# google-research/nerf-from-image

Measured on AMD Instinct MI355X. Metric: rendered rays/sec (128x128, 64+64 samples), higher is better.
Workload: dtype f32 (decoder MLP operands split-fp16 hi+lo, 22 bits; strict fp32: config.value_mlp_exact_fp32)

## Files before the change

### nerf_from_image_amd/csrc/nfi_kernels.hip

```cpp
#include "nfi_device.hpp"
#include "../../include/nfi_hip.h"
#include "nfi_host.hpp"

#include <algorithm>
#include <cstddef>
#include <cstdio>
#include <cstring>

using namespace nfi;

thread_local char nfi_err_buf[256] = "";
extern "C" const char* nfi_last_error(void) { return nfi_err_buf; }
extern "C" int nfi_version(void) { return 102; }


constexpr int kP2tPixels = 256, kP2tPitch = 288;
template <int TEX>
__global__ __launch_bounds__(256) void planes_to_texels_kernel(const float* __restrict__ planes, void* __restrict__ texels,
                                                               int hw) {
  __shared__ __attribute__((aligned(16))) float tile[kC][kP2tPitch];
  const int img = blockIdx.y;
  const int px0 = blockIdx.x * kP2tPixels;
  const float* src = planes + (size_t)img * kC * hw;
  {
// ... 1005 lines not shown
  const int64_t ray = (int64_t)blockIdx.x * 4 + wave;
  if (ray >= a.n_rays) return;
  WaveSlab& slab = slabs[wave];
  const int M = a.n_bins, K = a.n_samples;
  float bins[2], wts[2];
#pragma unroll
  for (int j = 0; j < 2; ++j) {
    int e = j * 64 + lane;
    bins[j] = e < M ? a.bins[ray * M + e] : 0.0f;
    wts[j] = e < M - 1 ? a.weights[ray * (M - 1) + e] : 0.0f;
  }
  build_cdf<2>(slab, bins, wts, M, lane);
#pragma unroll
  for (int j = 0; j < 2; ++j) {
    int e = j * 64 + lane;
    if (e < K) {
      float u = a.u[ray * a.u_row_stride + e];
      int ind;
      float z = invert_cdf<16>(slab, M, u, ind);
      a.samples[ray * K + e] = z;
      if (a.inds) a.inds[ray * K + e] = ind;
    }
    if (a.cdf && e < M) a.cdf[ray * M + e] = slab.cdf[e];
  }
}

extern "C" int nfi_sample_pdf(const nfi_sample_pdf_args* a, nfi_stream_t stream) {
  REQUIRE(a && a->bins && a->weights && a->u && a->samples, "sample_pdf: null pointer");
  REQUIRE(a->n_rays > 0 && a->n_bins >= 2 && a->n_bins <= 128 && a->n_samples >= 1 && a->n_samples <= 128,
          "sample_pdf: need 2 <= bins <= 128 and 1 <= samples <= 128");
  hipLaunchKernelGGL(sample_pdf_kernel, dim3((unsigned)((a->n_rays + 3) / 4)), dim3(256), 0, (hipStream_t)stream, *a);
  return check_launch("sample_pdf");
}

__global__ __launch_bounds__(256) void resample_kernel(nfi_resample_args a) {
  __shared__ WaveSlab slabs[4];
  const int lane = lane_id();
  const int wave = threadIdx.x >> 6;
  const int64_t ray = (int64_t)blockIdx.x * 4 + wave;
  if (ray >= a.n_rays) return;
  WaveSlab& slab = slabs[wave];
  const int S = a.n_samples;
  float sigma = lane < S ? a.sigma[ray * S + lane] : 0.0f;
  float t = lane < S ? a.depth[ray * S + lane] : 0.0f;
  float u = lane < S ? a.u[ray * a.u_row_stride + lane] : 0.0f;
  float dn = norm3(a.ray_directions[ray * 3], a.ray_directions[ray * 3 + 1], a.ray_directions[ray * 3 + 2]);
  ResampleTaps taps;
  float z = resample_ray(slab, sigma, t, S, dn, u, lane, &taps);
  if (lane < S) {
    a.fine_depth[ray * S + lane] = z;
    if (a.weights) a.weights[ray * S + lane] = taps.w;
    if (a.smooth) a.smooth[ray * S + lane] = taps.smooth;
    if (a.inds) a.inds[ray * S + lane] = taps.ind;
  }
  if (a.cdf && lane < S - 1) a.cdf[ray * (S - 1) + lane] = slab.cdf[lane];
}

__global__ __launch_bounds__(256) void resample_wide_kernel(nfi_resample_args a) {
  __shared__ WaveSlab slabs[4];
  const int lane = lane_id();
  const int wave = threadIdx.x >> 6;
  const int64_t ray = (int64_t)blockIdx.x * 4 + wave;
  if (ray >= a.n_rays) return;
  WaveSlab& slab = slabs[wave];
  const int S = a.n_samples;
  float sigma[2], t[2], u[2], z[2], w[2], sm[2];
  int ind[2];
#pragma unroll
  for (int j = 0; j < 2; ++j) {
    const int e = j * 64 + lane;
    sigma[j] = e < S ? a.sigma[ray * S + e] : 0.0f;
    t[j] = e < S ? a.depth[ray * S + e] : 0.0f;
    u[j] = e < S ? a.u[ray * a.u_row_stride + e] : 0.0f;
  }
  float dn = norm3(a.ray_directions[ray * 3], a.ray_directions[ray * 3 + 1], a.ray_directions[ray * 3 + 2]);
  float Tc[2];
  resample_ray_wide<2>(slab, sigma, t, S, dn, u, lane, z, w, sm, ind, Tc);
#pragma unroll
  for (int j = 0; j < 2; ++j) {
    const int e = j * 64 + lane;
    if (e < S) {
      a.fine_depth[ray * S + e] = z[j];
      if (a.weights) a.weights[ray * S + e] = w[j];
      if (a.smooth) a.smooth[ray * S + e] = sm[j];
      if (a.inds) a.inds[ray * S + e] = ind[j];
    }
    if (a.cdf && e < S - 1) a.cdf[ray * (S - 1) + e] = slab.cdf[e];
  }
}

extern "C" int nfi_resample(const nfi_resample_args* a, nfi_stream_t stream) {
  REQUIRE(a && a->sigma && a->ray_directions && a->depth && a->u && a->fine_depth, "resample: null pointer");
  REQUIRE(a->n_rays > 0 && a->n_samples >= 4 && a->n_samples <= NFI_MAX_SAMPLES, "resample: n_samples must be in [4,128]");
  const dim3 grid((unsigned)((a->n_rays + 3) / 4));
  if (a->n_samples <= 64) hipLaunchKernelGGL(resample_kernel, grid, dim3(256), 0, (hipStream_t)stream, *a);
  else hipLaunchKernelGGL(resample_wide_kernel, grid, dim3(256), 0, (hipStream_t)stream, *a);
  return check_launch("resample");
}

template <int NS>
__global__ __launch_bounds__(256) void composite_kernel(nfi_composite_args a) {
  __shared__ WaveSlabT<64 * NS> slabs[4];
  const int lane = lane_id();
  const int wave = threadIdx.x >> 6;
  const int64_t ray = (int64_t)blockIdx.x * 4 + wave;
  if (ray >= a.n_rays) return;
  auto& slab = slabs[wave];
  const int na = a.n_a, nb = a.n_b, n = na + nb;
  float dep[NS], sig[NS], cr[NS], cg[NS], cb[NS];
  int eidx[NS];
#pragma unroll
  for (int j = 0; j < NS; ++j) {
    int e = j * 64 + lane;
    dep[j] = sig[j] = cr[j] = cg[j] = cb[j] = 0.0f;
    eidx[j] = e;
    if (e < na) {
      size_t i = (size_t)ray * na + e;
      dep[j] = a.depth_a[i]; sig[j] = a.sigma_a[i];
      cr[j] = a.rgb_a[i * 3]; cg[j] = a.rgb_a[i * 3 + 1]; cb[j] = a.rgb_a[i * 3 + 2];
    } else if (e < n) {
      size_t i = (size_t)ray * nb + (e - na);
      dep[j] = a.depth_b[i]; sig[j] = a.sigma_b[i];
      cr[j] = a.rgb_b[i * 3]; cg[j] = a.rgb_b[i * 3 + 1]; cb[j] = a.rgb_b[i * 3 + 2];
    }
  }
  int rank[NS];
  if (nb > 0) {
    merge_scatter<NS>(slab, dep, sig, cr, cg, cb, eidx, n, rank);
  } else {
#pragma unroll
    for (int j = 0; j < NS; ++j) {
      int e = j * 64 + lane;
      rank[j] = e;
      if (e < n) { slab.srt[0][e] = dep[j]; slab.srt[1][e] = sig[j]; slab.srt[2][e] = cr[j]; slab.srt[3][e] = cg[j]; slab.srt[4][e] = cb[j]; }
    }
    wave_lds_fence();
  }
  float dn = norm3(a.ray_directions[ray * 3], a.ray_directions[ray * 3 + 1], a.ray_directions[ray * 3 + 2]);
  float w[NS];
  CompositeOut o = composite_slab<NS>(slab, n, dn, a.white_background, lane, w);
  if (lane == 0) {
    a.rgb_map[ray * 3] = o.r; a.rgb_map[ray * 3 + 1] = o.g; a.rgb_map[ray * 3 + 2] = o.b;
    a.depth_map[ray] = o.depth;
    a.mask[ray] = o.mask;
  }
#pragma unroll
  for (int j = 0; j < NS; ++j) {
    int e = j * 64 + lane;
    if (e < n) {
      if (a.weights) a.weights[(size_t)ray * n + e] = w[j];
      if (a.depth_sorted) a.depth_sorted[(size_t)ray * n + e] = slab.srt[0][e];
      if (a.perm) a.perm[(size_t)ray * n + rank[j]] = e;
    }
  }
  if (a.n_extra > 0 && a.extra_map) {
    wave_lds_fence();
#pragma unroll
    for (int j = 0; j < NS; ++j) {
      int e = j * 64 + lane;
      if (e < n) slab.cdf[e] = w[j];
    }
    wave_lds_fence();
    float we[NS];
#pragma unroll
    for (int j = 0; j < NS; ++j) { int e = j * 64 + lane; we[j] = e < n ? slab.cdf[rank[j]] : 0.0f; }
    for (int c = 0; c < a.n_extra; ++c) {
      float acc = 0.0f;
#pragma unroll
      for (int j = 0; j < NS; ++j) {
        int e = j * 64 + lane;
        if (e < na) acc += we[j] * a.extra_a[((size_t)ray * na + e) * a.n_extra + c];
        else if (e < n) acc += we[j] * a.extra_b[((size_t)ray * nb + (e - na)) * a.n_extra + c];
      }
      acc = wave_sum(acc);
      if (lane == 0) a.extra_map[ray * a.n_extra + c] = acc;
    }
  }
}

extern "C" int nfi_composite_fwd(const nfi_composite_args* a, nfi_stream_t stream) {
  REQUIRE(a && a->ray_directions && a->depth_a && a->sigma_a && a->rgb_a && a->rgb_map && a->depth_map && a->mask,
          "composite: null pointer");
  REQUIRE(a->n_rays > 0 && a->n_a > 0 && a->n_b >= 0 && a->n_a + a->n_b <= NFI_MAX_SAMPLES_SINGLE_PASS,
          "composite: need 1 <= n_a + n_b <= 512");
  REQUIRE(a->n_b == 0 || (a->n_a <= NFI_MAX_SAMPLES && a->n_b <= NFI_MAX_SAMPLES), "composite: merged lists hold at most 128 samples each");
  REQUIRE(a->n_b == 0 || (a->depth_b && a->sigma_b && a->rgb_b), "composite: list b missing");
  REQUIRE(a->n_extra == 0 || (a->extra_a && (a->n_b == 0 || a->extra_b)), "composite: extra attribute missing");
  const dim3 grid((unsigned)((a->n_rays + 3) / 4));
  if (a->n_a + a->n_b <= 128) hipLaunchKernelGGL(composite_kernel<2>, grid, dim3(256), 0, (hipStream_t)stream, *a);
  else if (a->n_a + a->n_b <= 256) hipLaunchKernelGGL(composite_kernel<4>, grid, dim3(256), 0, (hipStream_t)stream, *a);
  else hipLaunchKernelGGL(composite_kernel<8>, grid, dim3(256), 0, (hipStream_t)stream, *a);
  return check_launch("composite_fwd");
}

#include "nfi_backward_rays.inc"
#include "nfi_regulariser.inc"
#include "nfi_neighbours.inc"
#include "nfi_handoff.inc"
#include "nfi_pnp.inc"
#include "nfi_viewdir_mapper.inc"

struct RenderKernelParams {
  int n_scenes, hw, S;
  int fine, white;
  float scene_range;
  const float* ro; const float* rd; const float* near_raw; const float* far_raw; const uint8_t* hit;
  const uint32_t* reduce;
  uint32_t* counter;
  int width;
  int tile_order;
  int xcd_blocks;
  uint32_t* xcd_counter;
  int xcd_block_shift;
  int fetch_batch;
  const void* texels; int res; int layout;
  const float* image; int A; const float* att;
  int use_sdf; const float* beta; const float* alpha;
  const float* noise_c; const float* noise_f; int64_t noise_f_stride;
  float* rgb; float* depth; float* mask;
  float* near_plane; float* far_plane;
  float* t_coarse; float* sigma_coarse; float* rgb_coarse;
  float* t_fine; float* sigma_fine; float* rgb_fine;
  float* t_sorted; float* weights; int32_t* perm;
  int skip_missed;
  unsigned long long* prof;
  const float* xray;
  float term_eps;
  float* semantics;
  float* coords;
  float* normals;
  unsigned long long* clock_probe;
  FastDiv div_scene_rays, div_bps, div_bw;
  int tap_stride;
  int stash;
};

struct ClockProbe {
  unsigned long long c0 = 0, r0 = 0;
  bool on = false;
  __device__ __forceinline__ void start(const RenderKernelParams& k) {
    on = k.clock_probe && blockIdx.x == 0 && threadIdx.x == 0;
    if (on) { c0 = __builtin_readcyclecounter(); r0 = __builtin_amdgcn_s_memrealtime(); }
  }
  __device__ __forceinline__ void stop(const RenderKernelParams& k) const {
    if (on) {
      k.clock_probe[0] = __builtin_readcyclecounter() - c0;
      k.clock_probe[1] = __builtin_amdgcn_s_memrealtime() - r0;
    }
  }
};

__device__ __forceinline__ float uniform_f32(float v) {
  return bits2f((uint32_t)__builtin_amdgcn_readfirstlane((int)f2bits(v)));
}

struct RayInputs {
  float ox, oy, oz, dx, dy, dz, near, far, noise, u;
  uint32_t hit;
};

struct RayQueue {
  const RenderKernelParams& k;
  int lane;
  uint32_t n_rays, xcd, bsh, bw, bps, n_blocks, q_cur, pos_next, pos_end, batch, tiles_x;
  bool dry;
  __device__ __forceinline__ RayQueue(const RenderKernelParams& kk, int l) : k(kk), lane(l) {
    n_rays = (uint32_t)k.n_scenes * (uint32_t)k.hw;
    xcd = k.xcd_blocks ? (__builtin_amdgcn_s_getreg(6164) & 7u) : 0u;
    bsh = (uint32_t)k.xcd_block_shift;
    bw = (uint32_t)k.width >> bsh;
    bps = bw * (((uint32_t)k.hw / (uint32_t)k.width) >> bsh);
    n_blocks = bps * (uint32_t)k.n_scenes;
    q_cur = xcd; pos_next = 0; pos_end = 0; dry = false;
    batch = (uint32_t)k.fetch_batch;
    tiles_x = (uint32_t)k.width >> 3;
  }
  __device__ __forceinline__ uint32_t ray_at(uint32_t q, uint32_t pos) const {
    const uint32_t b = (pos >> (2 * bsh)) * 8u + q;
    const uint32_t in = pos & ((1u << (2 * bsh)) - 1u), scene = fastdiv(b, k.div_bps), bb = b - scene * bps;
    const uint32_t by = fastdiv(bb, k.div_bw), bx = bb - by * bw;
    const uint32_t st = in >> 6, sty = st >> (bsh - 3), stx = st & ((1u << (bsh - 3)) - 1u);
    const uint32_t y = (by << bsh) + (sty << 3) + ((in >> 3) & 7u), x = (bx << bsh) + (stx << 3) + (in & 7u);
    return scene * (uint32_t)k.hw + y * (uint32_t)k.width + x;
  }
  __device__ __forceinline__ uint32_t fetch() {
    if (!k.xcd_blocks) {
      uint32_t p = 0;
      if (lane == 0) p = atomicAdd(k.counter, 1u);
      return (uint32_t)__builtin_amdgcn_readfirstlane((int)p);
    }
    if (pos_next == pos_end && !dry) {
      dry = true;
      for (uint32_t i = 0; i < 8; ++i) {
        uint32_t base = 0;
        if (lane == 0) base = atomicAdd(k.xcd_counter + q_cur * 16, batch);
        base = (uint32_t)__builtin_amdgcn_readfirstlane((int)base);
        if ((base >> (2 * bsh)) * 8u + q_cur < n_blocks) { pos_next = base; pos_end = base + batch; dry = false; break; }
        q_cur = (q_cur + 1) & 7u;
      }
    }
    if (dry) return n_rays;
    return ray_at(q_cur, pos_next++);
  }
  __device__ __forceinline__ uint32_t ray_of(uint32_t pos) const {
    if (k.xcd_blocks || !k.tile_order) return pos;
    const uint32_t scene = pos / (uint32_t)k.hw, p = pos - scene * (uint32_t)k.hw;
    const uint32_t tile = p >> 6, in = p & 63u;
    const uint32_t ty = tile / tiles_x, tx = tile - ty * tiles_x;
    return scene * (uint32_t)k.hw + ((ty << 3) + (in >> 3)) * (uint32_t)k.width + (tx << 3) + (in & 7u);
  }
};

constexpr int kRenderPlain = 0, kRenderTaps = 1, kRenderProf = 2, kRenderTerm = 3, kRenderExtra = 4, kRenderNormals = 5;
constexpr int kSemPitch = 2 * 64 + 4;
constexpr int kSemPitchWide = 2 * 128 + 8;
extern __shared__ __attribute__((aligned(16))) float nfi_dyn_lds[];

typedef __attribute__((address_space(3))) float lds_float;

template <int NS, class Slab>
__device__ __forceinline__ void composite_coords(const Slab& slab, const float (&w)[NS], int n, int lane, float ox, float oy,
                                                 float oz, float dx, float dy, float dz, float* out3) {
  float cx = 0.0f, cy = 0.0f, cz = 0.0f;
#pragma unroll
  for (int j = 0; j < NS; ++j) {
    const int e = j * 64 + lane;
    if (e < n) {
      const float t = slab.srt[0][e];
      cx += w[j] * (ox + dx * t); cy += w[j] * (oy + dy * t); cz += w[j] * (oz + dz * t);
    }
  }
  cx = wave_sum(cx); cy = wave_sum(cy); cz = wave_sum(cz);
  if (lane == 0) { out3[0] = cx; out3[1] = cy; out3[2] = cz; }
}


template <int PREC, int kImg>
__device__ __forceinline__ void stage_decoder_image(float* lds, const float* image) {
  if (PREC == 1) {
    for (int i = threadIdx.x; i < kB1F; i += blockDim.x) lds[i] = image[kW1H + i];
    for (int i = kB1F + threadIdx.x; i < kLdsImageFloats; i += blockDim.x) lds[i] = image[i];
  } else {
    for (int i = threadIdx.x; i < kImg; i += blockDim.x) lds[i] = image[i];
  }
  __syncthreads();
}

template <int TEX>
__device__ __forceinline__ void enter_scene(FieldParams& P, const RenderKernelParams& k, float* vf, int scene, int lane) {
  const size_t tb = TEX == 0 ? 128 : 64;
  const char* tex_scene = reinterpret_cast<const char*>(k.texels) + (size_t)scene * 3 * k.res * k.res * tb;
  P.rsrc = __builtin_amdgcn_make_buffer_rsrc(const_cast<char*>(tex_scene), 0, (int)P.scene_bytes, 0x00020000);
  wave_lds_fence();
  {
    int c = lane & 3, row = lane >> 2;
    float v = 0.0f;
    if (k.att && c < 3 && row >= 1 && row <= k.A) v = k.att[((size_t)scene * k.A + (row - 1)) * 3 + c];
    vf[lane] = v;
  }
  wave_lds_fence();
}

__device__ __forceinline__ void store_pixel(const RenderKernelParams& k, uint32_t ray, float r, float g, float b, float depth,
                                            float mask) {
  k.rgb[(size_t)ray * 3] = r; k.rgb[(size_t)ray * 3 + 1] = g; k.rgb[(size_t)ray * 3 + 2] = b;
  k.depth[ray] = depth; k.mask[ray] = mask;
}

__device__ __forceinline__ void store_sample_tap(float* t_out, float* sigma_out, float* rgb_out, size_t i, float t, float sigma,
                                                 float r, float g, float b) {
  if (t_out) t_out[i] = t;
  if (sigma_out) sigma_out[i] = sigma;
  if (rgb_out) { float* q = rgb_out + i * 3; q[0] = r; q[1] = g; q[2] = b; }
}

template <int NS, class Slab>
__device__ __forceinline__ void store_sorted_taps(const RenderKernelParams& k, const Slab& slab, const float (&w)[NS], uint32_t ray,
                                                  int n, int lane) {
#pragma unroll
  for (int j = 0; j < NS; ++j) {
    const int e = j * 64 + lane;
    if (e < n) {
      if (k.weights) k.weights[(size_t)ray * n + e] = w[j];
      if (k.t_sorted) k.t_sorted[(size_t)ray * n + e] = slab.srt[0][e];
    }
  }
}

template <bool NRM>
__device__ __forceinline__ void zero_missed_maps(const RenderKernelParams& k, uint32_t ray, int lane, float bg) {
  if (k.coords && lane < 3) k.coords[(size_t)ray * 3 + lane] = 0.0f;
  if (k.semantics && lane < k.A) k.semantics[(size_t)ray * k.A + lane] = 0.0f;
  if (NRM && lane < 3) k.normals[(size_t)ray * 3 + lane] = bg;
}

__device__ __forceinline__ void zero_stash_row(const RenderKernelParams& k, uint32_t ray, int S, int lane) {
  for (int e = lane; e < S; e += 64) {
    const size_t zs = (size_t)ray * (size_t)k.tap_stride + e;
    k.t_coarse[zs] = 0.0f; k.sigma_coarse[zs] = 0.0f;
    float* q = k.rgb_coarse + zs * 3; q[0] = 0.0f; q[1] = 0.0f; q[2] = 0.0f;
    if (k.fine) {
      k.t_fine[zs] = 0.0f; k.sigma_fine[zs] = 0.0f;
      q = k.rgb_fine + zs * 3; q[0] = 0.0f; q[1] = 0.0f; q[2] = 0.0f;
    }
  }
}

template <int TEX, bool ATT, int OCC, int MODE, int PREC, bool VD = false>
__global__ __launch_bounds__(256, OCC) void render_fwd_kernel(RenderKernelParams k) {
  constexpr bool TAPS = MODE == kRenderTaps, PROF = MODE == kRenderProf, TERM = MODE == kRenderTerm;
  constexpr bool EXTRA = MODE == kRenderExtra || MODE == kRenderNormals, NRM = MODE == kRenderNormals;
  constexpr int SEMP = (EXTRA && ATT) ? kSemPitch : 0;
  constexpr int kImg = VD ? kVdImageFloats : kLdsImageFloats;
  __shared__ __attribute__((aligned(16))) float lds[kImg];
  __shared__ __attribute__((aligned(16))) float vfs[4][64];
  __shared__ WaveSlab slabs[4];
  if constexpr (NRM) stage_normal_operands(nfi_dyn_lds, k.image, VD ? kVdW1F : kW1F, VD ? kVdW2 : kW2F);
  ClockProbe clock;
  clock.start(k);
  stage_decoder_image<PREC, kImg>(lds, k.image);
  const int lane = lane_id();
  const int wave = threadIdx.x >> 6;
  WaveSlab& slab = slabs[wave];
  float* vf = vfs[wave];
  const int S = k.S;
  const bool valid = lane < S;
  const float fill_near = ordered_key_inv(~k.reduce[0]), fill_far = ordered_key_inv(k.reduce[1]);
  const float bg = k.white ? 1.0f : 0.0f;
  const uint32_t n_rays = (uint32_t)k.n_scenes * (uint32_t)k.hw;

  FieldParams P = make_field_params(k.texels, k.res, TEX, k.A, k.use_sdf, k.beta, k.alpha, lds, kImg, k.layout);
  P.vf = vf;
  P.w1t = nfi_dyn_lds; P.w2r0 = nfi_dyn_lds + kW1TFloats;
  int cur_scene = -1;

  float* semT = nullptr;
  if constexpr (SEMP > 0) {
    if (k.semantics) {
      semT = nfi_dyn_lds + (NRM ? kNrmLdsFloats : 0) + wave * (k.A * kSemPitch);
      for (int i = lane; i < k.A * kSemPitch; i += 64) ((lds_float*)semT)[i] = 0.0f;
      wave_lds_fence();
    }
  }

  auto load_inputs = [&](uint32_t ray, RayInputs& in) {
    const size_t r3 = (size_t)ray * 3;
    in.hit = k.hit[ray];
    in.ox = k.ro[r3]; in.oy = k.ro[r3 + 1]; in.oz = k.ro[r3 + 2];
    in.dx = k.rd[r3]; in.dy = k.rd[r3 + 1]; in.dz = k.rd[r3 + 2];
    in.near = k.near_raw[ray]; in.far = k.far_raw[ray];
    in.noise = (k.noise_c && valid) ? k.noise_c[(size_t)ray * S + lane] : 0.0f;
    in.u = (k.fine && valid) ? k.noise_f[(size_t)ray * k.noise_f_stride + lane] : 0.0f;
  };

  RayQueue queue(k, lane);
  auto fetch = [&]() -> uint32_t { return queue.fetch(); };
  uint32_t cur = fetch(), nxt = fetch(), fly = 0;
  RayInputs in, pre;
  unsigned long long pc[12] = {0, 0, 0, 0, 0, 0, 0, 0, 0, 0, 0, 0};
  unsigned long long tk0 = PROF ? __builtin_readcyclecounter() : 0;
  if (cur < n_rays) load_inputs(queue.ray_of(cur), in);
  while (cur < n_rays) {
    if (nxt < n_rays) load_inputs(queue.ray_of(nxt), pre);
    const uint32_t ray = queue.ray_of(cur);
    const uint32_t hitb = in.hit;
    float out_r = bg, out_g = bg, out_b = bg, out_d = 0.0f, out_m = 0.0f;
    if (k.skip_missed && !(hitb & 2)) {
      if constexpr (EXTRA) zero_missed_maps<NRM>(k, ray, lane, bg);
      if constexpr (TAPS) {
        if (k.stash) zero_stash_row(k, ray, S, lane);
      }
    } else {
      unsigned long long t0 = PROF ? __builtin_readcyclecounter() : 0;
      const int scene = (int)fastdiv(ray, k.div_scene_rays);
      if (scene != cur_scene) {
        cur_scene = scene;
        enter_scene<TEX>(P, k, vf, scene, lane);
      }
      const float ox = in.ox, oy = in.oy, oz = in.oz, dx = in.dx, dy = in.dy, dz = in.dz;
      float near = in.near, far = in.far;
      finish_planes((hitb & 1) != 0, fill_near, fill_far, near, far);
      const float dnorm = norm3(dx, dy, dz);
      const size_t rs = (size_t)ray * (size_t)k.tap_stride;

      float tc = 0.0f;
      if (valid) tc = stratified_depth(near, far, lane, S, in.noise, k.noise_c != nullptr);
      MergeIn c;
      float ncx = 0.0f, ncy = 0.0f, ncz = 0.0f, nfx = 0.0f, nfy = 0.0f, nfz = 0.0f;
      unsigned long long t1 = PROF ? __builtin_readcyclecounter() : 0;
      {
        SampleOut q = field_wave<TEX, ATT, true, PREC, VD, SEMP, NRM>(P, k.scene_range, lane, ox + dx * tc, oy + dy * tc, oz + dz * tc,
                                                                      valid, semT, nullptr, &slab.srt[0][0], PROF ? pc : nullptr,
                                                                      k.xray, (int)ray);
        c.t = tc; c.sigma = q.sigma; c.r = q.r; c.g = q.g; c.b = q.b;
        if constexpr (NRM) { ncx = q.nx; ncy = q.ny; ncz = q.nz; }
      }
      int n = S;
      int rank_c = lane, rank_f = 0;
      unsigned long long t2 = PROF ? __builtin_readcyclecounter() : 0, t3 = t2, t4 = t2, t5 = t2;
      if (k.fine) {
        ResampleTaps rt;
        float tf = resample_ray(slab, c.sigma, tc, S, dnorm, in.u, lane, TERM ? &rt : nullptr);
        MergeIn f;
        if (PROF) { asm volatile("" :: "v"(tf)); t3 = __builtin_readcyclecounter(); }
        if constexpr (TERM) {
          const uint64_t dm = __ballot(valid && rt.T < k.term_eps);
          float t_dead = INFINITY;
          if (dm) t_dead = bits2f((uint32_t)__builtin_amdgcn_readlane((int)f2bits(tc), (int)__builtin_ctzll(dm)));
          const bool live = valid && tf <= t_dead;
          const uint64_t lm = __ballot(live);
          const int nl = __builtin_popcountll(lm);
          const int nb = __builtin_popcountll(lm & ((1ull << lane) - 1ull));
          const int pos = live ? nb : nl + (lane - nb);
          wave_lds_fence();
          slab.cdf[pos] = tf;
          wave_lds_fence();
          tf = slab.cdf[lane];
          wave_lds_fence();
          const bool vl = lane < nl;
          SampleOut q = field_wave<TEX, ATT, true, PREC, VD>(P, k.scene_range, lane, ox + dx * tf, oy + dy * tf, oz + dz * tf, vl,
                                                             nullptr, nullptr, &slab.srt[0][0], nullptr, k.xray, (int)ray);
          f.t = tf; f.sigma = vl ? q.sigma : 0.0f; f.r = vl ? q.r : 0.0f; f.g = vl ? q.g : 0.0f; f.b = vl ? q.b : 0.0f;
        } else {
          SampleOut q = field_wave<TEX, ATT, true, PREC, VD, SEMP, NRM>(P, k.scene_range, lane, ox + dx * tf, oy + dy * tf, oz + dz * tf,
                                                                        valid, semT ? semT + 64 : nullptr, nullptr, &slab.srt[0][0],
                                                                        PROF ? pc : nullptr, k.xray, (int)ray);
          f.t = tf; f.sigma = q.sigma; f.r = q.r; f.g = q.g; f.b = q.b;
          if constexpr (NRM) { nfx = q.nx; nfy = q.ny; nfz = q.nz; }
        }
        if constexpr (TAPS) {
          if (valid) store_sample_tap(k.t_fine, k.sigma_fine, k.rgb_fine, rs + lane, tf, f.sigma, f.r, f.g, f.b);
        }
        n = 2 * S;
        if (PROF) t4 = __builtin_readcyclecounter();
        merge_pair_scatter(slab, c, f, S, lane, rank_c, rank_f);
        if (PROF) t5 = __builtin_readcyclecounter();
      } else {
        if (valid) { slab.srt[0][lane] = c.t; slab.srt[1][lane] = c.sigma; slab.srt[2][lane] = c.r; slab.srt[3][lane] = c.g; slab.srt[4][lane] = c.b; }
        wave_lds_fence();
      }
      float w[2];
      CompositeOut o = composite_slab<2>(slab, n, dnorm, k.white, lane, w);
      out_r = o.r; out_g = o.g; out_b = o.b; out_d = o.depth; out_m = o.mask;
      if constexpr (EXTRA) {
        if (k.coords) composite_coords<2>(slab, w, n, lane, ox, oy, oz, dx, dy, dz, k.coords + (size_t)ray * 3);
        float wc = 0.0f, wf = 0.0f;
        if ((SEMP > 0 && semT) || NRM) {
          wave_lds_fence();
          slab.cdf[lane] = w[0]; slab.cdf[64 + lane] = w[1];
          wave_lds_fence();
          wc = valid ? slab.cdf[rank_c] : 0.0f;
          wf = (valid && k.fine) ? slab.cdf[rank_f] : 0.0f;
        }
        if constexpr (NRM) {
          const float bgn = k.white ? 1.0f - o.mask : 0.0f;
          const float mx = wave_sum(wc * ncx + wf * nfx) + bgn, my = wave_sum(wc * ncy + wf * nfy) + bgn,
                      mz = wave_sum(wc * ncz + wf * nfz) + bgn;
          if (lane == 0) { float* q = k.normals + (size_t)ray * 3; q[0] = mx; q[1] = my; q[2] = mz; }
        }
        if constexpr (SEMP > 0) {
          if (semT) {
            const lds_float* sl = (const lds_float*)semT;
            float mine = 0.0f;
            for (int a = 0; a < k.A; ++a) {
              const float sa = wave_sum(wc * sl[a * kSemPitch + lane] + wf * sl[a * kSemPitch + 64 + lane]);
              if (lane == a) mine = sa;
            }
            if (lane < k.A) k.semantics[(size_t)ray * k.A + lane] = mine;
          }
        }
      }
      if constexpr (TAPS) {
        if (lane == 0) {
          if (k.near_plane) k.near_plane[ray] = near;
          if (k.far_plane) k.far_plane[ray] = far;
        }
        if (valid) {
          store_sample_tap(k.t_coarse, k.sigma_coarse, k.rgb_coarse, rs + lane, tc, c.sigma, c.r, c.g, c.b);
          if (k.perm) {
            k.perm[(size_t)ray * n + rank_c] = lane;
            if (k.fine) k.perm[(size_t)ray * n + rank_f] = S + lane;
          }
        }
        store_sorted_taps<2>(k, slab, w, ray, n, lane);
      }
      wave_lds_fence();
      if (PROF) {
        unsigned long long t6 = __builtin_readcyclecounter();
        pc[4] += t1 - t0; pc[5] += t2 - t1; pc[6] += t3 - t2; pc[7] += t4 - t3; pc[8] += t5 - t4; pc[9] += t6 - t5; pc[10] += 1;
      }
    }
    fly = fetch();
    if (lane == 0) store_pixel(k, ray, out_r, out_g, out_b, out_d, out_m);
    in = pre;
    cur = nxt;
    nxt = fly;
  }
  if (PROF && k.prof && lane == 0) {
    pc[11] = __builtin_readcyclecounter() - tk0;
    for (int i = 0; i < 12; ++i) atomicAdd(k.prof + i, pc[i]);
  }
  clock.stop(k);
}

#ifdef NFI_SINGLE_KERNEL
#ifndef NFI_SINGLE_MODE
#define NFI_SINGLE_MODE 0
#endif
template __global__ void render_fwd_kernel<NFI_SINGLE_KERNEL, true, NFI_RENDER_OCC, NFI_SINGLE_MODE, 1>(RenderKernelParams);
#endif
#if !defined(NFI_SINGLE_KERNEL) || defined(NFI_SINGLE_WIDE)
template <int TEX, bool ATT, int MODE, int PREC, bool VD = false, int OCC = NFI_RENDER_OCC>
__global__ __launch_bounds__(256, OCC) void render_fwd_wide_kernel(RenderKernelParams k) {
  constexpr bool TAPS = MODE == kRenderTaps, TERM = MODE == kRenderTerm;
  constexpr bool EXTRA = MODE == kRenderExtra || MODE == kRenderNormals, NRM = MODE == kRenderNormals;
  constexpr int SEMP = (EXTRA && ATT) ? -kSemPitchWide : 0;
  constexpr int kImg = VD ? kVdImageFloats : kLdsImageFloats;
  __shared__ __attribute__((aligned(16))) float lds[kImg];
  __shared__ __attribute__((aligned(16))) float vfs[4][64];
  __shared__ WaveSlabWide slabs[4];
  if constexpr (NRM) stage_normal_operands(nfi_dyn_lds, k.image, VD ? kVdW1F : kW1F, VD ? kVdW2 : kW2F);
  ClockProbe clock;
  clock.start(k);
  stage_decoder_image<PREC, kImg>(lds, k.image);
  const int lane = lane_id();
  const int wave = threadIdx.x >> 6;
  WaveSlabWide& slab = slabs[wave];
  float* vf = vfs[wave];
  const int S = k.S;
  const float fill_near = ordered_key_inv(~k.reduce[0]), fill_far = ordered_key_inv(k.reduce[1]);
  const float bg = k.white ? 1.0f : 0.0f;
  const uint32_t n_rays = (uint32_t)k.n_scenes * (uint32_t)k.hw;
  FieldParams P = make_field_params(k.texels, k.res, TEX, k.A, k.use_sdf, k.beta, k.alpha, lds, kImg, k.layout);
  P.vf = vf;
  P.w1t = nfi_dyn_lds; P.w2r0 = nfi_dyn_lds + kW1TFloats;
  int cur_scene = -1;
  typedef __attribute__((address_space(3))) unsigned short lds_u16;
  float* semT = nullptr;
  if constexpr (SEMP != 0) {
    if (k.semantics) {
      semT = reinterpret_cast<float*>(reinterpret_cast<unsigned short*>(nfi_dyn_lds + (NRM ? kNrmLdsFloats : 0)) +
                                      wave * (k.A * kSemPitchWide));
      for (int i = lane; i < k.A * kSemPitchWide / 2; i += 64) ((lds_float*)semT)[i] = 0.0f;
      wave_lds_fence();
    }
  }
  auto sem_col = [&](int c) -> float* {
    return semT ? reinterpret_cast<float*>(reinterpret_cast<unsigned short*>(semT) + c) : nullptr;
  };
  RayQueue queue(k, lane);
  uint32_t cur = queue.fetch(), nxt = 0;
  while (cur < n_rays) {
    nxt = queue.fetch();
    const uint32_t ray = queue.ray_of(cur);
    const uint32_t hitb = k.hit[ray];
    if (k.skip_missed && !(hitb & 2)) {
      if (lane == 0) store_pixel(k, ray, bg, bg, bg, 0.0f, 0.0f);
      if constexpr (EXTRA) zero_missed_maps<NRM>(k, ray, lane, bg);
      if constexpr (TAPS) {
        if (k.stash) zero_stash_row(k, ray, S, lane);
      }
    } else {
      const int scene = (int)fastdiv(ray, k.div_scene_rays);
      if (scene != cur_scene) {
        cur_scene = scene;
        enter_scene<TEX>(P, k, vf, scene, lane);
      }
      const size_t r3 = (size_t)ray * 3;
      const float ox = k.ro[r3], oy = k.ro[r3 + 1], oz = k.ro[r3 + 2];
      const float dx = k.rd[r3], dy = k.rd[r3 + 1], dz = k.rd[r3 + 2];
      float near = k.near_raw[ray], far = k.far_raw[ray];
      finish_planes((hitb & 1) != 0, fill_near, fill_far, near, far);
      const float dnorm = norm3(dx, dy, dz);
      const size_t rs = (size_t)ray * S;
      const size_t ts = (size_t)ray * (size_t)k.tap_stride;
      float* stage = &slab.srt[0][0];

      float tc[2], sc[2], rc[2], gc[2], bc[2];
      bool val[2];
#pragma unroll
      for (int j = 0; j < 2; ++j) {
        const int e = j * 64 + lane;
        val[j] = e < S;
        const float nz = (k.noise_c && val[j]) ? k.noise_c[rs + e] : 0.0f;
        tc[j] = val[j] ? stratified_depth(near, far, e, S, nz, k.noise_c != nullptr) : 0.0f;
      }
      float nrm[4][3];
#pragma unroll
      for (int j = 0; j < 4; ++j) nrm[j][0] = nrm[j][1] = nrm[j][2] = 0.0f;
#pragma unroll
      for (int j = 0; j < 2; ++j) {
        SampleOut q = field_wave<TEX, ATT, true, PREC, VD, SEMP, NRM>(P, k.scene_range, lane, ox + dx * tc[j], oy + dy * tc[j],
                                                                      oz + dz * tc[j], val[j], sem_col(j * 64), nullptr,
                                                                      stage, nullptr, k.xray, (int)ray);
        sc[j] = q.sigma; rc[j] = q.r; gc[j] = q.g; bc[j] = q.b;
        if constexpr (NRM) { nrm[j][0] = q.nx; nrm[j][1] = q.ny; nrm[j][2] = q.nz; }
      }
      int n = S;
      float dep[4], sig[4], cr[4], cg[4], cb[4];
      int eidx[4], rank[4];
#pragma unroll
      for (int j = 0; j < 2; ++j) {
        dep[j] = tc[j]; sig[j] = sc[j]; cr[j] = rc[j]; cg[j] = gc[j]; cb[j] = bc[j];
        eidx[j] = val[j] ? j * 64 + lane : 0x7fffffff;
        dep[2 + j] = sig[2 + j] = cr[2 + j] = cg[2 + j] = cb[2 + j] = 0.0f;
        eidx[2 + j] = 0x7fffffff;
        rank[j] = j * 64 + lane; rank[2 + j] = 0;
      }
      if (k.fine) {
        float u[2], tf[2], wtap[2], smtap[2], Tc[2];
        int ind[2];
#pragma unroll
        for (int j = 0; j < 2; ++j) u[j] = val[j] ? k.noise_f[(size_t)ray * k.noise_f_stride + j * 64 + lane] : 0.0f;
        wave_lds_fence();
        resample_ray_wide<2>(slab, sc, tc, S, dnorm, u, lane, tf, wtap, smtap, ind, Tc);
        bool vfine[2] = {val[0], val[1]};
        if constexpr (TERM) {
          const uint64_t dm0 = __ballot(val[0] && Tc[0] < k.term_eps);
          const uint64_t dm1 = __ballot(val[1] && Tc[1] < k.term_eps);
          float t_dead = INFINITY;
          if (dm0) t_dead = bits2f((uint32_t)__builtin_amdgcn_readlane((int)f2bits(tc[0]), (int)__builtin_ctzll(dm0)));
          else if (dm1) t_dead = bits2f((uint32_t)__builtin_amdgcn_readlane((int)f2bits(tc[1]), (int)__builtin_ctzll(dm1)));
          const bool l0 = val[0] && tf[0] <= t_dead, l1 = val[1] && tf[1] <= t_dead;
          const uint64_t lm0 = __ballot(l0), lm1 = __ballot(l1);
          const int n0 = __builtin_popcountll(lm0), nl = n0 + __builtin_popcountll(lm1);
          const uint64_t below = (1ull << lane) - 1ull;
          const int b0 = __builtin_popcountll(lm0 & below), b1 = __builtin_popcountll(lm1 & below);
          const int p0 = l0 ? b0 : nl + (lane - b0);
          const int p1 = l1 ? n0 + b1 : nl + (64 - n0) + (lane - b1);
          wave_lds_fence();
          slab.cdf[p0] = tf[0];
          slab.cdf[p1] = tf[1];
          wave_lds_fence();
          tf[0] = slab.cdf[lane];
          tf[1] = slab.cdf[64 + lane];
          wave_lds_fence();
          vfine[0] = lane < nl;
          vfine[1] = 64 + lane < nl;
        }
#pragma unroll
        for (int j = 0; j < 2; ++j) {
          SampleOut q = field_wave<TEX, ATT, true, PREC, VD, SEMP, NRM>(P, k.scene_range, lane, ox + dx * tf[j], oy + dy * tf[j],
                                                                        oz + dz * tf[j], vfine[j], sem_col(128 + j * 64),
                                                                        nullptr, stage, nullptr, k.xray, (int)ray);
          if (TERM && !vfine[j]) { q.sigma = 0.0f; q.r = 0.0f; q.g = 0.0f; q.b = 0.0f; }
          if constexpr (NRM) { nrm[2 + j][0] = q.nx; nrm[2 + j][1] = q.ny; nrm[2 + j][2] = q.nz; }
          dep[2 + j] = tf[j]; sig[2 + j] = q.sigma; cr[2 + j] = q.r; cg[2 + j] = q.g; cb[2 + j] = q.b;
          eidx[2 + j] = val[j] ? S + j * 64 + lane : 0x7fffffff;
          if constexpr (TAPS) {
            if (val[j]) store_sample_tap(k.t_fine, k.sigma_fine, k.rgb_fine, ts + j * 64 + lane, tf[j], q.sigma, q.r, q.g, q.b);
          }
        }
        n = 2 * S;
        wave_lds_fence();
        if (!merge_pair_scatter_wide(slab, dep, sig, cr, cg, cb, S, lane, rank))
          merge_scatter<4>(slab, dep, sig, cr, cg, cb, eidx, n, rank);
      } else {
        wave_lds_fence();
#pragma unroll
        for (int j = 0; j < 2; ++j) {
          const int e = j * 64 + lane;
          if (val[j]) { slab.srt[0][e] = tc[j]; slab.srt[1][e] = sc[j]; slab.srt[2][e] = rc[j]; slab.srt[3][e] = gc[j]; slab.srt[4][e] = bc[j]; }
        }
        wave_lds_fence();
      }
      float w[4];
      CompositeOut o = composite_slab<4>(slab, n, dnorm, k.white, lane, w);
      if (lane == 0) store_pixel(k, ray, o.r, o.g, o.b, o.depth, o.mask);
      if constexpr (EXTRA) {
        if (k.coords) composite_coords<4>(slab, w, n, lane, ox, oy, oz, dx, dy, dz, k.coords + (size_t)ray * 3);
        float ws[4] = {0.0f, 0.0f, 0.0f, 0.0f};
        if ((SEMP != 0 && semT) || NRM) {
          wave_lds_fence();
#pragma unroll
          for (int j = 0; j < 4; ++j) slab.cdf[j * 64 + lane] = w[j];
          wave_lds_fence();
#pragma unroll
          for (int j = 0; j < 2; ++j) {
            ws[j] = val[j] ? slab.cdf[rank[j]] : 0.0f;
            ws[2 + j] = (val[j] && k.fine) ? slab.cdf[rank[2 + j]] : 0.0f;
          }
        }
        if constexpr (NRM) {
          const float bgn = k.white ? 1.0f - o.mask : 0.0f;
          float m3[3];
#pragma unroll
          for (int c = 0; c < 3; ++c)
            m3[c] = wave_sum((ws[0] * nrm[0][c] + ws[1] * nrm[1][c]) + (ws[2] * nrm[2][c] + ws[3] * nrm[3][c])) + bgn;
          if (lane == 0) { float* q = k.normals + (size_t)ray * 3; q[0] = m3[0]; q[1] = m3[1]; q[2] = m3[2]; }
        }
        if constexpr (SEMP != 0) {
          if (semT) {
            const lds_u16* sl = (const lds_u16*)semT;
            float mine = 0.0f;
            for (int a = 0; a < k.A; ++a) {
              const lds_u16* row = sl + a * kSemPitchWide + lane;
              const float sa = wave_sum((ws[0] * (float)row[0] + ws[1] * (float)row[64]) + (ws[2] * (float)row[128] + ws[3] * (float)row[192]));
              if (lane == a) mine = sa * (1.0f / 65535.0f);
            }
            const float tot = wave_sum(mine);
            if (tot > 0.0f) mine *= o.mask / tot;
            if (lane < k.A) k.semantics[(size_t)ray * k.A + lane] = mine;
          }
        }
      }
      if constexpr (TAPS) {
        if (lane == 0) {
          if (k.near_plane) k.near_plane[ray] = near;
          if (k.far_plane) k.far_plane[ray] = far;
        }
#pragma unroll
        for (int j = 0; j < 2; ++j) {
          if (val[j]) {
            store_sample_tap(k.t_coarse, k.sigma_coarse, k.rgb_coarse, ts + j * 64 + lane, tc[j], sc[j], rc[j], gc[j], bc[j]);
            if (k.perm) {
              k.perm[(size_t)ray * n + rank[j]] = j * 64 + lane;
              if (k.fine) k.perm[(size_t)ray * n + rank[2 + j]] = S + j * 64 + lane;
            }
          }
        }
        store_sorted_taps<4>(k, slab, w, ray, n, lane);
      }
      wave_lds_fence();
    }
    cur = nxt;
  }
  clock.stop(k);
}

#endif
#ifdef NFI_SINGLE_WIDE
template __global__ void render_fwd_wide_kernel<NFI_SINGLE_KERNEL, true, NFI_SINGLE_MODE, 1, false, NFI_RENDER_OCC>(RenderKernelParams);
#endif
#ifndef NFI_SINGLE_KERNEL
struct __attribute__((aligned(16))) WaveSlabLong {
  float srt[5][NFI_MAX_SAMPLES_SINGLE_PASS];
  float stage[16 * 36];
};

template <int TEX, bool ATT, int PREC, bool VD = false>
__global__ __launch_bounds__(256, NFI_RENDER_OCC) void render_fwd_long_kernel(RenderKernelParams k) {
  constexpr int kImg = VD ? kVdImageFloats : kLdsImageFloats;
  constexpr int NS = NFI_MAX_SAMPLES_SINGLE_PASS / 64;
  __shared__ __attribute__((aligned(16))) float lds[kImg];
  __shared__ __attribute__((aligned(16))) float vfs[4][64];
  __shared__ WaveSlabLong slabs[4];
  ClockProbe clock;
  clock.start(k);
  stage_decoder_image<PREC, kImg>(lds, k.image);
  const int lane = lane_id();
  const int wave = threadIdx.x >> 6;
  WaveSlabLong& slab = slabs[wave];
  float* vf = vfs[wave];
  const int S = k.S;
  const int slots = (S + 63) >> 6;
  const float fill_near = ordered_key_inv(~k.reduce[0]), fill_far = ordered_key_inv(k.reduce[1]);
  const float bg = k.white ? 1.0f : 0.0f;
  const uint32_t n_rays = (uint32_t)k.n_scenes * (uint32_t)k.hw;
  FieldParams P = make_field_params(k.texels, k.res, TEX, k.A, k.use_sdf, k.beta, k.alpha, lds, kImg, k.layout);
  P.vf = vf;
  int cur_scene = -1;
  RayQueue queue(k, lane);
  uint32_t cur = queue.fetch(), nxt = 0;
  while (cur < n_rays) {
    nxt = queue.fetch();
    const uint32_t ray = queue.ray_of(cur);
    const uint32_t hitb = k.hit[ray];
    const size_t ts = (size_t)ray * (size_t)k.tap_stride;
    if (k.skip_missed && !(hitb & 2)) {
      if (lane == 0) store_pixel(k, ray, bg, bg, bg, 0.0f, 0.0f);
      if (k.stash) zero_stash_row(k, ray, S, lane);
    } else {
      const int scene = (int)fastdiv(ray, k.div_scene_rays);
      if (scene != cur_scene) {
        cur_scene = scene;
        enter_scene<TEX>(P, k, vf, scene, lane);
      }
      const size_t r3 = (size_t)ray * 3;
      const float ox = k.ro[r3], oy = k.ro[r3 + 1], oz = k.ro[r3 + 2];
      const float dx = k.rd[r3], dy = k.rd[r3 + 1], dz = k.rd[r3 + 2];
      float near = k.near_raw[ray], far = k.far_raw[ray];
      finish_planes((hitb & 1) != 0, fill_near, fill_far, near, far);
      const float dnorm = norm3(dx, dy, dz);
      const size_t rs = (size_t)ray * S;
#pragma unroll 1
      for (int j = 0; j < slots; ++j) {
        const int e = j * 64 + lane;
        const bool val = e < S;
        const float nz = (k.noise_c && val) ? k.noise_c[rs + e] : 0.0f;
        const float t = val ? stratified_depth(near, far, e, S, nz, k.noise_c != nullptr) : 0.0f;
        SampleOut q = field_wave<TEX, ATT, true, PREC, VD>(P, k.scene_range, lane, ox + dx * t, oy + dy * t, oz + dz * t, val,
                                                           nullptr, nullptr, slab.stage, nullptr, k.xray, (int)ray);
        if (val) {
          slab.srt[0][e] = t; slab.srt[1][e] = q.sigma; slab.srt[2][e] = q.r; slab.srt[3][e] = q.g; slab.srt[4][e] = q.b;
          store_sample_tap(k.t_coarse, k.sigma_coarse, k.rgb_coarse, ts + e, t, q.sigma, q.r, q.g, q.b);
        }
      }
      wave_lds_fence();
      float w[NS];
// ... 297 lines not shown
```

Measured before the change: 146.7 million.

## Skip runs of missed rays with scalar hit checks and split queue claims

Missed rays (no bounding hit) are now handled in a dedicated loop that reads hit bytes for two rays at once through scalar loads, writes background outputs directly and keeps claiming rays until it finds one that needs rendering. The queue claim is split into issue and finish steps so the atomic can overlap with the background stores. The main render loop no longer carries a branch for missed rays. This adds queue state complexity and may change ordering or prefetch behaviour around scene transitions.

New measurement: 148.3 million, median of 6. 1.1% higher.

```diff
diff --git a/nerf_from_image_amd/csrc/nfi_kernels.hip b/nerf_from_image_amd/csrc/nfi_kernels.hip
--- a/nerf_from_image_amd/csrc/nfi_kernels.hip
+++ b/nerf_from_image_amd/csrc/nfi_kernels.hip
@@ -1331,6 +1331,24 @@
     if (dry) return n_rays;
     return ray_at(q_cur, pos_next++);
   }
+  __device__ __forceinline__ bool claimed() const { return pos_next != pos_end; }
+  __device__ __forceinline__ uint32_t take() { return ray_at(q_cur, pos_next++); }
+  __device__ __forceinline__ uint32_t claim_issue() const {
+    uint32_t raw = 0, off = k.xcd_blocks ? q_cur * 16 : 0;
+    asm volatile("" : "+v"(off));
+    if (k.xcd_blocks && (claimed() || dry)) return raw;
+    if (lane == 0) raw = atomicAdd((k.xcd_blocks ? k.xcd_counter : k.counter) + off, k.xcd_blocks ? batch : 1u);
+    return raw;
+  }
+  __device__ __forceinline__ uint32_t claim_finish(uint32_t raw) {
+    const uint32_t base = (uint32_t)__builtin_amdgcn_readfirstlane((int)raw);
+    if (!k.xcd_blocks) return base;
+    if (!claimed() && !dry) {
+      if ((base >> (2 * bsh)) * 8u + q_cur < n_blocks) { pos_next = base; pos_end = base + batch; }
+      else q_cur = (q_cur + 1) & 7u;
+    }
+    return fetch();
+  }
   __device__ __forceinline__ uint32_t ray_of(uint32_t pos) const {
     if (k.xcd_blocks || !k.tile_order) return pos;
     const uint32_t scene = pos / (uint32_t)k.hw, p = pos - scene * (uint32_t)k.hw;
@@ -1433,6 +1451,57 @@
       q = k.rgb_fine + zs * 3; q[0] = 0.0f; q[1] = 0.0f; q[2] = 0.0f;
     }
   }
+}
+
+template <bool EXTRA, bool NRM, bool TAPS>
+__device__ __forceinline__ void put_missed_ray(const RenderKernelParams& k, uint32_t ray, int S, int lane, float bg) {
+  if (lane == 0) store_pixel(k, ray, bg, bg, bg, 0.0f, 0.0f);
+  if constexpr (EXTRA) zero_missed_maps<NRM>(k, ray, lane, bg);
+  if constexpr (TAPS) {
+    if (k.stash) zero_stash_row(k, ray, S, lane);
+  }
+}
+
+__device__ __forceinline__ uint32_t hit_bytes_scalar(const RenderKernelParams& k, uint32_t ra, uint32_t rb) {
+  typedef __attribute__((address_space(4))) const uint32_t const_u32;
+  const uintptr_t pa = reinterpret_cast<uintptr_t>(k.hit) + (uint32_t)__builtin_amdgcn_readfirstlane((int)ra),
+                  pb = reinterpret_cast<uintptr_t>(k.hit) + (uint32_t)__builtin_amdgcn_readfirstlane((int)rb);
+  uint32_t wa = *reinterpret_cast<const_u32*>(pa & ~(uintptr_t)3), wb = *reinterpret_cast<const_u32*>(pb & ~(uintptr_t)3);
+  asm volatile("" : "+s"(wa), "+s"(wb));
+  return ((wa >> ((uint32_t)(pa & 3) * 8u)) & 0xffu) | (((wb >> ((uint32_t)(pb & 3) * 8u)) & 0xffu) << 8);
+}
+
+template <bool EXTRA, bool NRM, bool TAPS, class Load>
+__device__ __forceinline__ void skip_miss_run(RayQueue& queue, const RenderKernelParams& k, int S, int lane, float bg,
+                                              uint32_t& cur, uint32_t& nxt, Load&& load) {
+  put_missed_ray<EXTRA, NRM, TAPS>(k, queue.ray_of(cur), S, lane, bg);
+  uint32_t a = nxt;
+  while (a < queue.n_rays) {
+    const bool two = queue.claimed();
+    const uint32_t b = two ? queue.take() : a;
+    const uint32_t ra = queue.ray_of(a), rb = queue.ray_of(b);
+    const uint32_t hits = hit_bytes_scalar(k, ra, rb);
+    uint32_t claim;
+    bool ends = true;
+    if (hits & 2u) {
+      cur = a; load(ra);
+      if (two) { nxt = b; return; }
+      claim = queue.claim_issue();
+    } else if (two && (hits & 0x200u)) {
+      put_missed_ray<EXTRA, NRM, TAPS>(k, ra, S, lane, bg);
+      cur = b; load(rb);
+      claim = queue.claim_issue();
+    } else {
+      claim = queue.claim_issue();
+      put_missed_ray<EXTRA, NRM, TAPS>(k, ra, S, lane, bg);
+      if (two) put_missed_ray<EXTRA, NRM, TAPS>(k, rb, S, lane, bg);
+      ends = false;
+    }
+    const uint32_t got = queue.claim_finish(claim);
+    if (ends) { nxt = got; return; }
+    a = got;
+  }
+  cur = nxt = a;
 }
 
 template <int TEX, bool ATT, int OCC, int MODE, int PREC, bool VD = false>
@@ -1489,141 +1558,140 @@
   unsigned long long pc[12] = {0, 0, 0, 0, 0, 0, 0, 0, 0, 0, 0, 0};
   unsigned long long tk0 = PROF ? __builtin_readcyclecounter() : 0;
   if (cur < n_rays) load_inputs(queue.ray_of(cur), in);
+  auto skip_run = [&]() {
+    if (k.skip_missed && cur < n_rays && !((uint32_t)__builtin_amdgcn_readfirstlane((int)in.hit) & 2))
+      skip_miss_run<EXTRA, NRM, TAPS>(queue, k, S, lane, bg, cur, nxt, [&](uint32_t r) { load_inputs(r, in); });
+  };
+  skip_run();
   while (cur < n_rays) {
     if (nxt < n_rays) load_inputs(queue.ray_of(nxt), pre);
     const uint32_t ray = queue.ray_of(cur);
     const uint32_t hitb = in.hit;
     float out_r = bg, out_g = bg, out_b = bg, out_d = 0.0f, out_m = 0.0f;
-    if (k.skip_missed && !(hitb & 2)) {
-      if constexpr (EXTRA) zero_missed_maps<NRM>(k, ray, lane, bg);
+    unsigned long long t0 = PROF ? __builtin_readcyclecounter() : 0;
+    const int scene = (int)fastdiv(ray, k.div_scene_rays);
+    if (scene != cur_scene) {
+      cur_scene = scene;
+      enter_scene<TEX>(P, k, vf, scene, lane);
+    }
+    const float ox = in.ox, oy = in.oy, oz = in.oz, dx = in.dx, dy = in.dy, dz = in.dz;
+    float near = in.near, far = in.far;
+    finish_planes((hitb & 1) != 0, fill_near, fill_far, near, far);
+    const float dnorm = norm3(dx, dy, dz);
+    const size_t rs = (size_t)ray * (size_t)k.tap_stride;
+
+    float tc = 0.0f;
+    if (valid) tc = stratified_depth(near, far, lane, S, in.noise, k.noise_c != nullptr);
+    MergeIn c;
+    float ncx = 0.0f, ncy = 0.0f, ncz = 0.0f, nfx = 0.0f, nfy = 0.0f, nfz = 0.0f;
+    unsigned long long t1 = PROF ? __builtin_readcyclecounter() : 0;
+    {
+      SampleOut q = field_wave<TEX, ATT, true, PREC, VD, SEMP, NRM>(P, k.scene_range, lane, ox + dx * tc, oy + dy * tc, oz + dz * tc,
+                                                                    valid, semT, nullptr, &slab.srt[0][0], PROF ? pc : nullptr,
+                                                                    k.xray, (int)ray);
+      c.t = tc; c.sigma = q.sigma; c.r = q.r; c.g = q.g; c.b = q.b;
+      if constexpr (NRM) { ncx = q.nx; ncy = q.ny; ncz = q.nz; }
+    }
+    int n = S;
+    int rank_c = lane, rank_f = 0;
+    unsigned long long t2 = PROF ? __builtin_readcyclecounter() : 0, t3 = t2, t4 = t2, t5 = t2;
+    if (k.fine) {
+      ResampleTaps rt;
+      float tf = resample_ray(slab, c.sigma, tc, S, dnorm, in.u, lane, TERM ? &rt : nullptr);
+      MergeIn f;
+      if (PROF) { asm volatile("" :: "v"(tf)); t3 = __builtin_readcyclecounter(); }
+      if constexpr (TERM) {
+        const uint64_t dm = __ballot(valid && rt.T < k.term_eps);
+        float t_dead = INFINITY;
+        if (dm) t_dead = bits2f((uint32_t)__builtin_amdgcn_readlane((int)f2bits(tc), (int)__builtin_ctzll(dm)));
+        const bool live = valid && tf <= t_dead;
+        const uint64_t lm = __ballot(live);
+        const int nl = __builtin_popcountll(lm);
+        const int nb = __builtin_popcountll(lm & ((1ull << lane) - 1ull));
+        const int pos = live ? nb : nl + (lane - nb);
+        wave_lds_fence();
+        slab.cdf[pos] = tf;
+        wave_lds_fence();
+        tf = slab.cdf[lane];
+        wave_lds_fence();
+        const bool vl = lane < nl;
+        SampleOut q = field_wave<TEX, ATT, true, PREC, VD>(P, k.scene_range, lane, ox + dx * tf, oy + dy * tf, oz + dz * tf, vl,
+                                                           nullptr, nullptr, &slab.srt[0][0], nullptr, k.xray, (int)ray);
+        f.t = tf; f.sigma = vl ? q.sigma : 0.0f; f.r = vl ? q.r : 0.0f; f.g = vl ? q.g : 0.0f; f.b = vl ? q.b : 0.0f;
+      } else {
+        SampleOut q = field_wave<TEX, ATT, true, PREC, VD, SEMP, NRM>(P, k.scene_range, lane, ox + dx * tf, oy + dy * tf, oz + dz * tf,
+                                                                      valid, semT ? semT + 64 : nullptr, nullptr, &slab.srt[0][0],
+                                                                      PROF ? pc : nullptr, k.xray, (int)ray);
+        f.t = tf; f.sigma = q.sigma; f.r = q.r; f.g = q.g; f.b = q.b;
+        if constexpr (NRM) { nfx = q.nx; nfy = q.ny; nfz = q.nz; }
+      }
       if constexpr (TAPS) {
-        if (k.stash) zero_stash_row(k, ray, S, lane);
-      }
+        if (valid) store_sample_tap(k.t_fine, k.sigma_fine, k.rgb_fine, rs + lane, tf, f.sigma, f.r, f.g, f.b);
+      }
+      n = 2 * S;
+      if (PROF) t4 = __builtin_readcyclecounter();
+      merge_pair_scatter(slab, c, f, S, lane, rank_c, rank_f);
+      if (PROF) t5 = __builtin_readcyclecounter();
     } else {
-      unsigned long long t0 = PROF ? __builtin_readcyclecounter() : 0;
-      const int scene = (int)fastdiv(ray, k.div_scene_rays);
-      if (scene != cur_scene) {
-        cur_scene = scene;
-        enter_scene<TEX>(P, k, vf, scene, lane);
-      }
-      const float ox = in.ox, oy = in.oy, oz = in.oz, dx = in.dx, dy = in.dy, dz = in.dz;
-      float near = in.near, far = in.far;
-      finish_planes((hitb & 1) != 0, fill_near, fill_far, near, far);
-      const float dnorm = norm3(dx, dy, dz);
-      const size_t rs = (size_t)ray * (size_t)k.tap_stride;
-
-      float tc = 0.0f;
-      if (valid) tc = stratified_depth(near, far, lane, S, in.noise, k.noise_c != nullptr);
-      MergeIn c;
-      float ncx = 0.0f, ncy = 0.0f, ncz = 0.0f, nfx = 0.0f, nfy = 0.0f, nfz = 0.0f;
-      unsigned long long t1 = PROF ? __builtin_readcyclecounter() : 0;
-      {
-        SampleOut q = field_wave<TEX, ATT, true, PREC, VD, SEMP, NRM>(P, k.scene_range, lane, ox + dx * tc, oy + dy * tc, oz + dz * tc,
-                                                                      valid, semT, nullptr, &slab.srt[0][0], PROF ? pc : nullptr,
-                                                                      k.xray, (int)ray);
-        c.t = tc; c.sigma = q.sigma; c.r = q.r; c.g = q.g; c.b = q.b;
-        if constexpr (NRM) { ncx = q.nx; ncy = q.ny; ncz = q.nz; }
-      }
-      int n = S;
-      int rank_c = lane, rank_f = 0;
-      unsigned long long t2 = PROF ? __builtin_readcyclecounter() : 0, t3 = t2, t4 = t2, t5 = t2;
-      if (k.fine) {
-        ResampleTaps rt;
-        float tf = resample_ray(slab, c.sigma, tc, S, dnorm, in.u, lane, TERM ? &rt : nullptr);
-        MergeIn f;
-        if (PROF) { asm volatile("" :: "v"(tf)); t3 = __builtin_readcyclecounter(); }
-        if constexpr (TERM) {
-          const uint64_t dm = __ballot(valid && rt.T < k.term_eps);
-          float t_dead = INFINITY;
-          if (dm) t_dead = bits2f((uint32_t)__builtin_amdgcn_readlane((int)f2bits(tc), (int)__builtin_ctzll(dm)));
-          const bool live = valid && tf <= t_dead;
-          const uint64_t lm = __ballot(live);
-          const int nl = __builtin_popcountll(lm);
-          const int nb = __builtin_popcountll(lm & ((1ull << lane) - 1ull));
-          const int pos = live ? nb : nl + (lane - nb);
-          wave_lds_fence();
-          slab.cdf[pos] = tf;
-          wave_lds_fence();
-          tf = slab.cdf[lane];
-          wave_lds_fence();
-          const bool vl = lane < nl;
-          SampleOut q = field_wave<TEX, ATT, true, PREC, VD>(P, k.scene_range, lane, ox + dx * tf, oy + dy * tf, oz + dz * tf, vl,
-                                                             nullptr, nullptr, &slab.srt[0][0], nullptr, k.xray, (int)ray);
-          f.t = tf; f.sigma = vl ? q.sigma : 0.0f; f.r = vl ? q.r : 0.0f; f.g = vl ? q.g : 0.0f; f.b = vl ? q.b : 0.0f;
-        } else {
-          SampleOut q = field_wave<TEX, ATT, true, PREC, VD, SEMP, NRM>(P, k.scene_range, lane, ox + dx * tf, oy + dy * tf, oz + dz * tf,
-                                                                        valid, semT ? semT + 64 : nullptr, nullptr, &slab.srt[0][0],
-                                                                        PROF ? pc : nullptr, k.xray, (int)ray);
-          f.t = tf; f.sigma = q.sigma; f.r = q.r; f.g = q.g; f.b = q.b;
-          if constexpr (NRM) { nfx = q.nx; nfy = q.ny; nfz = q.nz; }
+      if (valid) { slab.srt[0][lane] = c.t; slab.srt[1][lane] = c.sigma; slab.srt[2][lane] = c.r; slab.srt[3][lane] = c.g; slab.srt[4][lane] = c.b; }
+      wave_lds_fence();
+    }
+    float w[2];
+    CompositeOut o = composite_slab<2>(slab, n, dnorm, k.white, lane, w);
+    out_r = o.r; out_g = o.g; out_b = o.b; out_d = o.depth; out_m = o.mask;
+    if constexpr (EXTRA) {
+      if (k.coords) composite_coords<2>(slab, w, n, lane, ox, oy, oz, dx, dy, dz, k.coords + (size_t)ray * 3);
+      float wc = 0.0f, wf = 0.0f;
+      if ((SEMP > 0 && semT) || NRM) {
+        wave_lds_fence();
+        slab.cdf[lane] = w[0]; slab.cdf[64 + lane] = w[1];
+        wave_lds_fence();
+        wc = valid ? slab.cdf[rank_c] : 0.0f;
+        wf = (valid && k.fine) ? slab.cdf[rank_f] : 0.0f;
+      }
+      if constexpr (NRM) {
+        const float bgn = k.white ? 1.0f - o.mask : 0.0f;
+        const float mx = wave_sum(wc * ncx + wf * nfx) + bgn, my = wave_sum(wc * ncy + wf * nfy) + bgn,
+                    mz = wave_sum(wc * ncz + wf * nfz) + bgn;
+        if (lane == 0) { float* q = k.normals + (size_t)ray * 3; q[0] = mx; q[1] = my; q[2] = mz; }
+      }
+      if constexpr (SEMP > 0) {
+        if (semT) {
+          const lds_float* sl = (const lds_float*)semT;
+          float mine = 0.0f;
+          for (int a = 0; a < k.A; ++a) {
+            const float sa = wave_sum(wc * sl[a * kSemPitch + lane] + wf * sl[a * kSemPitch + 64 + lane]);
+            if (lane == a) mine = sa;
+          }
+          if (lane < k.A) k.semantics[(size_t)ray * k.A + lane] = mine;
         }
-        if constexpr (TAPS) {
-          if (valid) store_sample_tap(k.t_fine, k.sigma_fine, k.rgb_fine, rs + lane, tf, f.sigma, f.r, f.g, f.b);
+      }
+    }
+    if constexpr (TAPS) {
+      if (lane == 0) {
+        if (k.near_plane) k.near_plane[ray] = near;
+        if (k.far_plane) k.far_plane[ray] = far;
+      }
+      if (valid) {
+        store_sample_tap(k.t_coarse, k.sigma_coarse, k.rgb_coarse, rs + lane, tc, c.sigma, c.r, c.g, c.b);
+        if (k.perm) {
+          k.perm[(size_t)ray * n + rank_c] = lane;
+          if (k.fine) k.perm[(size_t)ray * n + rank_f] = S + lane;
         }
-        n = 2 * S;
-        if (PROF) t4 = __builtin_readcyclecounter();
-        merge_pair_scatter(slab, c, f, S, lane, rank_c, rank_f);
-        if (PROF) t5 = __builtin_readcyclecounter();
-      } else {
-        if (valid) { slab.srt[0][lane] = c.t; slab.srt[1][lane] = c.sigma; slab.srt[2][lane] = c.r; slab.srt[3][lane] = c.g; slab.srt[4][lane] = c.b; }
-        wave_lds_fence();
-      }
-      float w[2];
-      CompositeOut o = composite_slab<2>(slab, n, dnorm, k.white, lane, w);
-      out_r = o.r; out_g = o.g; out_b = o.b; out_d = o.depth; out_m = o.mask;
-      if constexpr (EXTRA) {
-        if (k.coords) composite_coords<2>(slab, w, n, lane, ox, oy, oz, dx, dy, dz, k.coords + (size_t)ray * 3);
-        float wc = 0.0f, wf = 0.0f;
-        if ((SEMP > 0 && semT) || NRM) {
-          wave_lds_fence();
-          slab.cdf[lane] = w[0]; slab.cdf[64 + lane] = w[1];
-          wave_lds_fence();
-          wc = valid ? slab.cdf[rank_c] : 0.0f;
-          wf = (valid && k.fine) ? slab.cdf[rank_f] : 0.0f;
-        }
-        if constexpr (NRM) {
-          const float bgn = k.white ? 1.0f - o.mask : 0.0f;
-          const float mx = wave_sum(wc * ncx + wf * nfx) + bgn, my = wave_sum(wc * ncy + wf * nfy) + bgn,
-                      mz = wave_sum(wc * ncz + wf * nfz) + bgn;
-          if (lane == 0) { float* q = k.normals + (size_t)ray * 3; q[0] = mx; q[1] = my; q[2] = mz; }
-        }
-        if constexpr (SEMP > 0) {
-          if (semT) {
-            const lds_float* sl = (const lds_float*)semT;
-            float mine = 0.0f;
-            for (int a = 0; a < k.A; ++a) {
-              const float sa = wave_sum(wc * sl[a * kSemPitch + lane] + wf * sl[a * kSemPitch + 64 + lane]);
-              if (lane == a) mine = sa;
-            }
-            if (lane < k.A) k.semantics[(size_t)ray * k.A + lane] = mine;
-          }
-        }
-      }
-      if constexpr (TAPS) {
-        if (lane == 0) {
-          if (k.near_plane) k.near_plane[ray] = near;
-          if (k.far_plane) k.far_plane[ray] = far;
-        }
-        if (valid) {
-          store_sample_tap(k.t_coarse, k.sigma_coarse, k.rgb_coarse, rs + lane, tc, c.sigma, c.r, c.g, c.b);
-          if (k.perm) {
-            k.perm[(size_t)ray * n + rank_c] = lane;
-            if (k.fine) k.perm[(size_t)ray * n + rank_f] = S + lane;
-          }
-        }
-        store_sorted_taps<2>(k, slab, w, ray, n, lane);
-      }
-      wave_lds_fence();
-      if (PROF) {
-        unsigned long long t6 = __builtin_readcyclecounter();
-        pc[4] += t1 - t0; pc[5] += t2 - t1; pc[6] += t3 - t2; pc[7] += t4 - t3; pc[8] += t5 - t4; pc[9] += t6 - t5; pc[10] += 1;
-      }
+      }
+      store_sorted_taps<2>(k, slab, w, ray, n, lane);
+    }
+    wave_lds_fence();
+    if (PROF) {
+      unsigned long long t6 = __builtin_readcyclecounter();
+      pc[4] += t1 - t0; pc[5] += t2 - t1; pc[6] += t3 - t2; pc[7] += t4 - t3; pc[8] += t5 - t4; pc[9] += t6 - t5; pc[10] += 1;
     }
     fly = fetch();
     if (lane == 0) store_pixel(k, ray, out_r, out_g, out_b, out_d, out_m);
     in = pre;
     cur = nxt;
     nxt = fly;
+    skip_run();
   }
   if (PROF && k.prof && lane == 0) {
     pc[11] = __builtin_readcyclecounter() - tk0;
```
